# xwhan/ProQA

Hardware: AMD Instinct MI355X
Metric: queries/sec top-80 MIPS over 18M x 128 index (higher is better)
Workload: dtype int8 nomination + f16 re-scoring; 1 GPU; top-80 MIPS, 2032 q x 18000000 x 128 fp16 rows in HBM (BASELINE configs[2]; x1 row shards: co...; rows=18000000, queries=2032, topk=80, parallelism=corpus-row-shard x1, exchange=none, rounds=4, fallback_rounds=0, leap_rank=33, world_size=1

## Files before the change

### proqa_amd/csrc/mips_index.cpp

```cpp
#include <algorithm>
#include <cmath>
#include <cstdio>
#include <cstdlib>
#include <cstring>
#include <condition_variable>
#include <mutex>
#include <new>
#include <thread>
#include <vector>

#include <fcntl.h>
#include <unistd.h>
#include <cerrno>

#include "common.h"
#include "mips_kernels.h"

namespace proqa {

struct Slab {
  long long r0, r1;
};

}
// ... 119 lines not shown
  } pending;
};

namespace proqa {
namespace {

constexpr int kMaxRounds = kOverflowWords;

bool debug_flag(const char* name) { return getenv(name) != nullptr; }
const bool kDebugCand = debug_flag("PROQA_DEBUG_CAND");
const unsigned kFilterFlags = getenv("PROQA_FILTER_FLAGS") ? (unsigned)atoi(getenv("PROQA_FILTER_FLAGS")) : 0u;
const int kWideQw = getenv("PROQA_FILTER_QW") && (atoi(getenv("PROQA_FILTER_QW")) == 4 || atoi(getenv("PROQA_FILTER_QW")) == 1)
                        ? atoi(getenv("PROQA_FILTER_QW")) : 2;
const bool kDebugRounds = debug_flag("PROQA_DEBUG_ROUNDS");
const bool kDeepRing = getenv("PROQA_I8_DEEP_RING") && atoi(getenv("PROQA_I8_DEEP_RING")) != 0;
const bool kRowSplit = !(getenv("PROQA_I8_ROW_SPLIT") && atoi(getenv("PROQA_I8_ROW_SPLIT")) == 0);
const double kSmallMergeLimit = getenv("PROQA_NOM_SMALL_MERGE_LIMIT") ? atof(getenv("PROQA_NOM_SMALL_MERGE_LIMIT")) : 200.0;

int read_inexact(proqa_index* idx, const char* what, hipStream_t st, unsigned* n_inexact) {
  unsigned c[2] = {0, 0};
  PROQA_HIP(hipMemcpyAsync(c, idx->inexact, sizeof c, hipMemcpyDeviceToHost, st));
  PROQA_HIP(hipStreamSynchronize(st));
  if (c[1])
    return fail(PROQA_EINVAL, "%s: %u float32 values exceed the fp16 range (|x| > 65504); such embeddings are not "
                              "supported", what, c[1]);
  *n_inexact = c[0];
  return PROQA_OK;
}

int reserve_rows32(proqa_index* idx, int64_t rows) {
// ... 106 lines not shown
  if (idx->xb8) (void)hipFree(idx->xb8);
      idx->xb8 = nullptr;
      idx->q8_epoch = idx->rows_epoch;
      return PROQA_OK;
    }
    idx->capacity8 = cap;
  }
  PROQA_HIP(hipMemsetAsync(idx->qstats, 0, sizeof(QuantStats), st));
  PROQA_HIP(launch_column_stats(idx->xb, idx->n, idx->col_partial, idx->col, idx->qstats, st));
  PROQA_HIP(launch_quantise_rows_i8(idx->xb, idx->n, idx->col, idx->xb8, idx->blk8, idx->qstats, st));
  QuantStats h;
  PROQA_HIP(hipMemcpyAsync(&h, idx->qstats, sizeof h, hipMemcpyDeviceToHost, st));
  PROQA_HIP(hipStreamSynchronize(st));
  idx->q8_epoch = idx->rows_epoch;
  idx->q8_usable = h.nonfinite == 0u && h.max_inorm != 0u;
  return PROQA_OK;
}

constexpr int64_t kAddPieceRows = 1 << 20;
constexpr int kLoaderSlots = 4;
constexpr int64_t kLoaderPieceBytes = 8 << 20;

int ingest_f32_piece(proqa_index* idx, int64_t row, int64_t m, const void* src_host, bool pinned, hipStream_t st) {
  if (int rc = ensure_stage(idx, (size_t)kAddPieceRows * kDim * 4)) return rc;
  char* dst = idx->xb + (size_t)row * kDim * 2;
  if (pinned)
    PROQA_HIP(hipMemcpyAsync(idx->stage_dev, src_host, (size_t)m * kDim * 4, hipMemcpyHostToDevice, st));
  else
    PROQA_HIP(hipMemcpy(idx->stage_dev, src_host, (size_t)m * kDim * 4, hipMemcpyHostToDevice));
  PROQA_HIP(hipMemsetAsync(idx->inexact, 0, 2 * sizeof(unsigned), st));
// ... 1182 lines not shown
  PROQA_HIP(hipEventRecord(idx->ev[0], st));
  int fallback = 0;
  auto prep_first = [&]() -> int {
    const bool check_q = dtype == PROQA_F32;
    if (check_q) PROQA_HIP(hipMemsetAsync(idx->inexact, 0, 2 * sizeof(unsigned), st));
    PROQA_HIP(launch_prep_queries(xq_dev, dtype, nq, idx->ws_nq_pad, idx->xq_pad, idx->tau, idx->run_n, idx->stat_dev,
                                  nullptr, true, check_q ? idx->inexact : nullptr, idx->overflow, st, idx->short_rounds));
    if (check_q) {
      unsigned bad = 0;
      if (int rc = read_inexact(idx, "index_search (queries)", st, &bad)) return rc;
      if (bad && !idx->allow_rounding)
        if (int rc = enable_exact(idx, st)) return rc;
    }
    return PROQA_OK;
  };
  auto setup_nominate = [&]() -> int {
    if (!nomination_eligible(idx, k)) return PROQA_OK;
    if (idx->q8_epoch != idx->rows_epoch) {
      if (idx->q8_searches_on_copy > 1) idx->q8_short_lived_builds = 0;
      if (idx->nominate_mode == 1 && idx->q8_short_lived_builds >= 2 && idx->q8_seen_epoch != idx->rows_epoch) {
        idx->q8_seen_epoch = idx->rows_epoch;
        log_line("index %p: rows changed again after an int8 copy that served %d search(es): this search scans the fp16 rows, the "
                 "copy is rebuilt when the rows stay", (void*)idx, idx->q8_searches_on_copy);
        return PROQA_OK;
      }
      idx->q8_seen_epoch = idx->rows_epoch;
      if (defer) {
        idx->q8_build_due = true;
        return PROQA_OK;
      }
      if (int rc = ensure_q8(idx, st)) return rc;
    }
    if (!idx->q8_usable) return PROQA_OK;
    if (idx->q8_unprofitable && idx->nominate_mode != 2) {
      if (++idx->q8_suspended_searches < idx->q8_probe_after) return PROQA_OK;
      log_line("index %p: re-probing the int8 nomination scan after %d searches on the fp16 rows", (void*)idx,
               idx->q8_suspended_searches);
    }
    PROQA_HIP(launch_prep_queries_i8(idx->xq_pad, idx->ws_nq_pad, idx->col, idx->qstats, idx->xq8, idx->qparams, idx->stat_nom, st));
    idx->q8_active = true;
    ++idx->q8_searches_on_copy;
    return PROQA_OK;
  };
  if (one_pass.use) {
    if (int rc = prep_first()) return rc;
    bool done = false;
    if (!idx->exact)
      if (int rc = search_one_pass(idx, one_pass, qw, n_qtiles, nq, nq_pad, k, PageOut{D_dev, (long long*)I_dev, idx_offset, k, 0},
                                   st, &done))
        return rc;
    if (done) {
      idx->stats.candidates += (int64_t)idx->mirror->candidates;
      (void)hipEventElapsedTime(&idx->stats.total_ms, idx->ev[0], idx->ev[1]);
      return PROQA_OK;
    }
    if (!idx->exact) ++fallback;
  }
  const int n_pages = ceil_div<int>(k, page_size);
  if (defer && n_pages == 1 && !fallback) {
    if (int rc = prep_first()) return rc;
    if (idx->exact)
      PROQA_HIP(launch_query_margins(xq_dev, dtype, nq, idx->ws_nq_pad, idx->norm_stats, idx->xq32, idx->margin,
                                     idx->tau, idx->tau_filter, st));
    if (int rc = setup_nominate()) return rc;
    PagePlan plan;
    if (int rc = page_enqueue(idx, qw, n_qtiles, nq, nq_pad, k, false, PageOut{D_dev, (long long*)I_dev, idx_offset, k, 0}, st, true,
                              &plan, status_dev))
      return rc;
    proqa_index::Pending& pe = idx->pending;
    pe.active = true;
    pe.qw = qw;
    pe.n_qtiles = n_qtiles;
    pe.nq = nq;
    pe.nq_pad = nq_pad;
    pe.k = k;
    pe.dtype = dtype;
    pe.xq_dev = xq_dev;
    pe.D = D_dev;
    pe.I = (long long*)I_dev;
    pe.idx_offset = idx_offset;
    pe.st = st;
    pe.slabs.swap(plan.slabs);
    pe.boot = plan.boot;
    return PROQA_OK;
  }
  if (n_pages > 1) PROQA_HIP(hipMemsetAsync(idx->done, 0, (size_t)idx->ws_nq_pad, st));
  for (int p = 0; p < n_pages; ++p) {
    const int page_k = std::min(page_size, k - p * page_size);
    if (p == 0) {
      if (int rc = prep_first()) return rc;
      if (n_pages == 1 && !fallback)
        if (int rc = setup_nominate()) return rc;
    } else {
      PROQA_HIP(launch_prep_queries(xq_dev, dtype, nq, idx->ws_nq_pad, idx->xq_pad, idx->tau, idx->run_n, idx->stat_dev,
                                    idx->done, false, nullptr, idx->overflow, st));
    }
    if (idx->exact)
      PROQA_HIP(launch_query_margins(xq_dev, dtype, nq, idx->ws_nq_pad, idx->norm_stats, idx->xq32, idx->margin,
                                     idx->tau, idx->tau_filter, st));
    const PageOut out{D_dev, (long long*)I_dev, idx_offset, k, p * page_size};
    bool boot_overflow = false;
    if (int rc = search_page(idx, qw, n_qtiles, nq, nq_pad, page_k, p > 0, out, st, &fallback, true, &boot_overflow)) return rc;
    if (boot_overflow) {
      PROQA_HIP(launch_prep_queries(xq_dev, dtype, nq, idx->ws_nq_pad, idx->xq_pad, idx->tau, idx->run_n, idx->stat_dev,
                                    nullptr, true, nullptr, idx->overflow, st));
      ++fallback;
      if (int rc = search_page(idx, qw, n_qtiles, nq, nq_pad, page_k, false, out, st, &fallback, false, &boot_overflow))
// ... 480 lines not shown
  if ((long long)n_parts * k >= (1ll << 27))
    return fail(PROQA_EINVAL, "topk_merge_device: n_parts*k=%lld is too large", (long long)n_parts * k);
  if (stride_d < nq * k || stride_i < nq * k)
    return fail(PROQA_EINVAL, "topk_merge_device: part strides %lld / %lld are shorter than a part (%lld)", (long long)stride_d,
                (long long)stride_i, (long long)(nq * k));
  PROQA_HIP(launch_merge_lists(D_parts_dev, (const long long*)I_parts_dev, n_parts, nq, k, (long long)stride_d, (long long)stride_i,
                               D_dev, (long long*)I_dev, as_stream(stream), nullptr, 0, nullptr, false));
  return PROQA_OK;
}

int proqa_topk_merge_device(const float* D_parts_dev, const int64_t* I_parts_dev, int n_parts, int64_t nq,
                            int k, float* D_dev, int64_t* I_dev, void* stream) {
  return proqa_topk_merge_strided_device(D_parts_dev, I_parts_dev, n_parts, nq, k, nq * k, nq * k, D_dev, I_dev, stream);
}

}
```

### proqa_amd/csrc/mips_kernels.h

```cpp
#pragma once
#include <hip/hip_runtime.h>
#include <stdint.h>

#include "../../include/proqa_hip.h"

namespace proqa {

constexpr int kDim = PROQA_EMBED_DIM;
constexpr int kFilterWaves = 8;
constexpr int kFilterThreads = kFilterWaves * 64;
__host__ __device__ constexpr unsigned filter_tile_queries(int qw) { return (qw == 4 ? 4u : 8u) * (unsigned)qw * 32u; }
constexpr int kStageRows = 128;
constexpr int kMergeThreads = 256;
constexpr int kMaxMergeListKeys = 16384;
constexpr int kMaxSortKeys = 2048;
constexpr int kPageK = kMaxSortKeys / 2;
constexpr int kBigSortKeys = 8192;
constexpr int kMidSortKeys = 4096;
constexpr int kBigPageK = kBigSortKeys / 2;
constexpr int kOnePassSortKeys = 16384;
constexpr int kOnePassMergeThreads = 1024;
constexpr int kOnePassLaneCap = 24;
constexpr int kLaneCap = 8;
constexpr int kBigLaneCap = 32;
// ... 65 lines not shown
  int compact;
  int nom_keys;
  const void* xq16;
  const char* xb16;
  unsigned long long* stat_nominated;
  int next_rank;
  int leap_check;
  unsigned* short_rounds;
  int round_bit;
};

constexpr int kStageBytesI8 = kStageRows * kDim;
struct NominateParams {
  float off;
  float inv_unit;
  float margin_r;
  float err_norm;
};
static_assert(sizeof(NominateParams) == 16, "one 16-byte load per lane");
struct QuantStats {
  unsigned max_resid;
  unsigned max_inorm;
  unsigned max_xnorm;
  unsigned nonfinite;
};
struct FilterArgsI8 {
  const signed char* xq8;
  const signed char* xb8;
  long long slab_row0;
  long long slab_row1;
  int rows_per_chunk;
  const float* tau;
  const NominateParams* qp;
  const float2* blk;
  CandidateStore store;
  unsigned* overflow;
  unsigned flags;
  unsigned q_blocks;
};
hipError_t launch_filter_i8(const FilterArgsI8& a, int qw, unsigned grid, hipStream_t st, bool deep = false);
constexpr int kColStatGroups = 1024;
hipError_t launch_column_stats(const void* xb16, long long n, float* partial, float* col, QuantStats* stats, hipStream_t st);
hipError_t launch_quantise_rows_i8(const void* xb16, long long n, const float* col, signed char* xb8, float2* blk, QuantStats* stats,
                                   hipStream_t st);
hipError_t launch_prep_queries_i8(const void* xq_pad16, long long nq_pad, const float* col, const QuantStats* stats,
                                  signed char* xq8, NominateParams* qp, unsigned long long* stat_nom, hipStream_t st);

hipError_t launch_filter(const FilterArgs& a, int qw, bool inclusive, unsigned grid, hipStream_t st);
#ifdef PROQA_FILTER_STAMPS
void read_filter_stamps(unsigned long long* out5);
#endif
hipError_t launch_advance_page(const unsigned long long* run_keys, const unsigned* run_n, long long nq, int page_k,
                               unsigned long long* bound_keys, float* ub, unsigned char* done, const float* margin,
                               float* ub_filter, hipStream_t st);
hipError_t launch_merge(const MergeArgs& a, unsigned nq_pad, hipStream_t st);
hipError_t launch_gather_index_rows(const void* xb16, const float* xb32, long long n_index, const long long* ids, long long n,
                                    long long idx_offset, void* out, bool out_f32, hipStream_t st);
hipError_t launch_flag_short_lists(const unsigned* run_n, long long nq, unsigned want, unsigned* flag, hipStream_t st);
hipError_t launch_bootstrap(const char* xb, const void* xq_pad, int n_rows, unsigned nq_pad, int k, float* scores,
                            unsigned long long* run_keys, unsigned* run_n, float* tau, unsigned long long* stat,
                            unsigned* overflow, hipStream_t st, int run_stride = 0, int tau_rank = 0);
// ... 42 lines not shown
```

### proqa_amd/csrc/mips_kernels.hip

```cpp
#include <hip/hip_runtime.h>
#include <algorithm>
#include <hipcub/hipcub.hpp>
#include <stdint.h>
#include <stdlib.h>

#include <type_traits>

#include "common.h"
#include "mips_kernels.h"

namespace proqa {
namespace {

typedef _Float16 f16x8 __attribute__((ext_vector_type(8)));
typedef float f32x16 __attribute__((ext_vector_type(16)));
typedef float f32x4 __attribute__((ext_vector_type(4)));

constexpr int kRowBytes = kDim * 2;
constexpr int kStageBytes = kStageRows * kRowBytes;
constexpr int kSubRows = 32;
#ifndef PROQA_DMA_AUX
#define PROQA_DMA_AUX 2
#endif
constexpr int kDmaAux = PROQA_DMA_AUX;
// ... 411 lines not shown
}

typedef int i32x4 __attribute__((ext_vector_type(4)));
typedef int i32x16 __attribute__((ext_vector_type(16)));
constexpr int kRowBytesI8 = kDim;
constexpr int kSubBytesI8 = kSubRows * kRowBytesI8;

__device__ __forceinline__ int imax(int a, int b) { return a > b ? a : b; }
__device__ __forceinline__ int max16_i32(const i32x16& v) {
  const int m0 = imax(imax(v[0], v[1]), v[2]), m1 = imax(imax(v[3], v[4]), v[5]), m2 = imax(imax(v[6], v[7]), v[8]),
            m3 = imax(imax(v[9], v[10]), v[11]), m4 = imax(imax(v[12], v[13]), v[14]);
  return imax(imax(imax(m0, m1), m2), imax(imax(m3, m4), v[15]));
}

struct LaneThreshold {
  float A, B, E;
};
__device__ __forceinline__ LaneThreshold lane_threshold(float tau, const NominateParams& p) {
  LaneThreshold t;
  t.B = p.margin_r;
  t.E = p.err_norm;
  if (!(tau > -__builtin_inff())) {
    t.A = -__builtin_inff();
  } else if (tau == __builtin_inff()) {
    t.A = __builtin_inff();
  } else {
    const float a = (tau - p.off) * p.inv_unit;
    t.A = a - __builtin_fabsf(a) * 0x1p-20f;
  }
  return t;
}
__device__ __forceinline__ float block_threshold(const LaneThreshold& t, float G, float X) {
  return __builtin_fmaf(-t.E, X, __builtin_fmaf(t.A, G, -t.B));
}

__device__ __forceinline__ unsigned nominee_mask(const i32x16& acc, float thr) {
  const int ti = thr < -2147483000.f ? (int)0x80000000 : (int)__builtin_floorf(thr);
  unsigned mask = 0u;
#define PROQA_BIT(n) "v_cmp_gt_i32 vcc, %" #n ", %17\n\tv_addc_co_u32 %0, vcc, %0, %0, vcc\n\t"
  asm volatile(PROQA_BIT(16) PROQA_BIT(15) PROQA_BIT(14) PROQA_BIT(13) PROQA_BIT(12) PROQA_BIT(11) PROQA_BIT(10) PROQA_BIT(9)
               PROQA_BIT(8) PROQA_BIT(7) PROQA_BIT(6) PROQA_BIT(5) PROQA_BIT(4) PROQA_BIT(3) PROQA_BIT(2) PROQA_BIT(1)
               : "+v"(mask)
               : "v"(acc[0]), "v"(acc[1]), "v"(acc[2]), "v"(acc[3]), "v"(acc[4]), "v"(acc[5]), "v"(acc[6]), "v"(acc[7]), "v"(acc[8]),
                 "v"(acc[9]), "v"(acc[10]), "v"(acc[11]), "v"(acc[12]), "v"(acc[13]), "v"(acc[14]), "v"(acc[15]), "v"(ti)
               : "vcc");
#undef PROQA_BIT
  return mask;
}
// ... 315 lines not shown
    const float* p = partial + (size_t)g * 3 * kDim;
    sum += (double)p[d];
    lo = __builtin_fminf(lo, p[kDim + d]);
    hi = __builtin_fmaxf(hi, p[2 * kDim + d]);
  }
  const float mean = (float)(sum / (double)(n > 0 ? n : 1));
  const float c = __builtin_fmaxf(hi - mean, mean - lo);
  const bool finite = c >= 0.f && c < __builtin_inff() && mean == mean;
  const float inv = finite && c > 0.f ? 1.0f / c : 0.f;
  if (!finite || !(inv < __builtin_inff())) atomicOr(&stats->nonfinite, 1u);
  col[d] = finite ? mean : 0.f;
  col[kDim + d] = inv;
  col[2 * kDim + d] = finite ? c : 0.f;
}

__global__ __launch_bounds__(256) void quantise_rows_i8(const _Float16* __restrict__ xb, long long n, const float* __restrict__ col,
                                                        signed char* __restrict__ xb8, float2* __restrict__ blk,
                                                        QuantStats* __restrict__ stats) {
  const int lane = threadIdx.x & 63;
  const int sub = lane & 15, rsub = lane >> 4;
  float mu[8], inv[8];
#pragma unroll
  for (int e = 0; e < 8; ++e) {
    mu[e] = col[sub * 8 + e];
    inv[e] = col[kDim + sub * 8 + e];
  }
  float max_r = 0.f, max_i = 0.f, max_x = 0.f;
  const long long n_blocks = (n + 31) / 32;
  for (long long b = (long long)blockIdx.x * 4 + (threadIdx.x >> 6); b < n_blocks; b += (long long)gridDim.x * 4) {
    float u[8][8];
    float amax = 0.f, sx_max = 0.f;
#pragma unroll
    for (int it = 0; it < 8; ++it) {
      const long long row = b * 32 + it * 4 + rsub;
      f16x8 v = {0};
      const bool live = row < n;
      if (live) v = *(const f16x8*)(xb + row * kDim + sub * 8);
      float sx = 0.f;
#pragma unroll
      for (int e = 0; e < 8; ++e) {
        const float x = (float)v[e];
        u[it][e] = live ? (x - mu[e]) * inv[e] : 0.f;
// ... 20 lines not shown
        const float i = __builtin_fminf(127.f, __builtin_fmaxf(-127.f, __builtin_rintf(t)));
        const float r = t - i;
        o[e] = (signed char)(int)i;
        sr += r * r;
        si += i * i;
      }
      if (row < n) *(i8x8*)(xb8 + row * kDim + sub * 8) = o;
#pragma unroll
      for (int off = 8; off > 0; off >>= 1) {
        sr += __shfl_xor(sr, off, 64);
        si += __shfl_xor(si, off, 64);
      }
      sr_max = sr > sr_max ? sr : sr_max;
      si_max = si > si_max ? si : si_max;
    }
    const float xb_ = __builtin_sqrtf(wave_max_f(si_max)) * (1.0f + 0x1p-10f);
    if (lane == 0) blk[b] = make_float2(G, xb_);
    max_r = sr_max > max_r ? sr_max : max_r;
    max_i = si_max > max_i ? si_max : max_i;
    max_x = sx_max > max_x ? sx_max : max_x;
  }
  max_r = wave_max_f(max_r);
  max_i = wave_max_f(max_i);
  max_x = wave_max_f(max_x);
  if (lane == 0) {
    const float r = __builtin_sqrtf(max_r) * (1.0f + 0x1p-10f), i = __builtin_sqrtf(max_i) * (1.0f + 0x1p-10f),
                x = __builtin_sqrtf(max_x) * (1.0f + 0x1p-10f);
    if (r > 0.f) atomicMax(&stats->max_resid, __float_as_uint(r));
    if (i > 0.f) atomicMax(&stats->max_inorm, __float_as_uint(i));
    if (x > 0.f) atomicMax(&stats->max_xnorm, __float_as_uint(x));
  }
}

__global__ __launch_bounds__(256) void prep_queries_i8(const _Float16* __restrict__ xq, long long nq_pad, const float* __restrict__ col,
                                                       const QuantStats* __restrict__ stats, signed char* __restrict__ xq8,
                                                       NominateParams* __restrict__ qp, unsigned long long* __restrict__ stat_nom) {
  const int lane = threadIdx.x & 63;
  const long long q = (long long)blockIdx.x * 4 + (threadIdx.x >> 6);
  if (q >= nq_pad) return;
  const float q0 = (float)xq[q * kDim + 2 * lane], q1 = (float)xq[q * kDim + 2 * lane + 1];
  const float mu0 = col[2 * lane], mu1 = col[2 * lane + 1];
  const float w0 = q0 * col[2 * kDim + 2 * lane], w1 = q1 * col[2 * kDim + 2 * lane + 1];
  const float wmax = wave_max_f(__builtin_fmaxf(__builtin_fabsf(w0), __builtin_fabsf(w1)));
  const float s_q = wmax / 127.0f;
  const bool ok = s_q > 0.f && s_q < __builtin_inff();
  const float inv = ok ? 1.0f / s_q : 0.f;
  const float u0 = w0 * inv, u1 = w1 * inv;
  const float i0 = __builtin_fminf(127.f, __builtin_fmaxf(-127.f, __builtin_rintf(u0)));
  const float i1 = __builtin_fminf(127.f, __builtin_fmaxf(-127.f, __builtin_rintf(u1)));
  typedef signed char i8x2 __attribute__((ext_vector_type(2)));
  const i8x2 o = {(signed char)(int)i0, (signed char)(int)i1};
  *(i8x2*)(xq8 + q * kDim + 2 * lane) = o;
  const float e0 = u0 - i0, e1 = u1 - i1;
  const float n_u = __builtin_sqrtf(wave_sum_f(u0 * u0 + u1 * u1)) * (1.0f + 0x1p-10f);
  const float n_e = __builtin_sqrtf(wave_sum_f(e0 * e0 + e1 * e1)) * (1.0f + 0x1p-10f) + 0x1p-10f;
  const float n_q = __builtin_sqrtf(wave_sum_f(q0 * q0 + q1 * q1)) * (1.0f + 0x1p-10f);
  const float abs_off = wave_sum_f(__builtin_fabsf(q0 * mu0) + __builtin_fabsf(q1 * mu1));
  double off = (double)q0 * (double)mu0 + (double)q1 * (double)mu1;
#pragma unroll
  for (int d = 32; d > 0; d >>= 1) off += __shfl_xor(off, d, 64);
  if (lane == 0) {
    const float R = __uint_as_float(stats->max_resid) + 0x1p-10f, Xf = __uint_as_float(stats->max_xnorm);
    const float delta = 0x1p-14f * n_q * Xf + 0x1p-20f * abs_off;
    NominateParams p;
    p.off = (float)off + delta + __builtin_fabsf((float)off) * 0x1p-22f;
    p.inv_unit = inv;
    p.margin_r = n_u * R * (1.0f + 0x1p-10f) + 0x1p-6f;
    p.err_norm = n_e;
    if (!(stats->nonfinite == 0u)) p.margin_r = __builtin_inff();
    qp[q] = p;
    stat_nom[q] = 0ull;
  }
}

__device__ __forceinline__ float filter_threshold(float t, float margin) {
  if (!(t > -__builtin_inff())) return t;
  return t - margin - __builtin_fabsf(t) * 0x1p-21f;
}

struct ExactCtx {
  unsigned* nom;
  unsigned* n_nom;
};

__device__ __forceinline__ void keep_scores_regs(const uint4 (&src)[5], unsigned q, bool inclusive,
                                                 unsigned long long bound, const ExactCtx& ex,
                                                 unsigned long long* keys, unsigned* n_keys, unsigned cap) {
// ... 765 lines not shown
  unsigned n = s_n_keys;
  if (n > kCompactKeys) {
    if (tid == 0) *a.overflow = 1u;
    n = kCompactKeys;
  }
  unsigned long long* dst = (unsigned long long*)(a.out.lane_log + lane_list_index(a.out, g >> 1, q, (int)(g & 1)) * a.out.lane_cap);
  if ((unsigned)tid < n) dst[tid] = s_keys[tid];
  if (tid == 0) {
    a.out.lane_cnt[lane_cnt_index(a.out, g >> 1, q, (int)(g & 1))] = n;
    if (a.stat_nominated) atomicAdd(a.stat_nominated + q, (unsigned long long)n_nom);
  }
}

constexpr int kBootWaves = 4;
constexpr int kBootTilesPerWave = 4;
__global__ __launch_bounds__(kBootWaves * 64) void bootstrap_scores(const char* __restrict__ xb, const void* __restrict__ xq,
                                                                    int n_rows, int s_stride, float* __restrict__ S) {
  __shared__ float tile[kBootWaves][32][33];
  const int lane = threadIdx.x & 63;
  const int wave = __builtin_amdgcn_readfirstlane(threadIdx.x >> 6);
  const int li = lane & 31, half = lane >> 5;
  const unsigned q0 = blockIdx.y * 32;
  const char* bp = (const char*)xq + (size_t)(q0 + li) * kRowBytes;
  f16x8 qf[8];
#pragma unroll
  for (int j = 0; j < 8; ++j) qf[j] = *(const f16x8*)(bp + (2 * j + half) * 16);
  f16x8 af[kBootTilesPerWave][8];
#pragma unroll
  for (int t = 0; t < kBootTilesPerWave; ++t) {
    const int row0 = ((blockIdx.x * kBootTilesPerWave + t) * kBootWaves + wave) * 32;
    const int arow = row0 + li < n_rows ? row0 + li : n_rows - 1;
    const char* ap = xb + (size_t)arow * kRowBytes;
#pragma unroll
    for (int j = 0; j < 8; ++j) af[t][j] = *(const f16x8*)(ap + (2 * j + half) * 16);
  }
#pragma unroll
  for (int t = 0; t < kBootTilesPerWave; ++t) {
    const int row0 = ((blockIdx.x * kBootTilesPerWave + t) * kBootWaves + wave) * 32;
    if (row0 >= n_rows) break;
    f32x16 acc = {0};
#pragma unroll
    for (int j = 0; j < 8; ++j) acc = __builtin_amdgcn_mfma_f32_32x32x16_f16(af[t][j], qf[j], acc, 0, 0, 0);
#pragma unroll
    for (int r = 0; r < 16; ++r) tile[wave][li][(r & 3) + 8 * (r >> 2) + 4 * half] = acc[r];
#pragma unroll
    for (int i = 0; i < 16; ++i) {
      const int qq = 2 * i + half;
      if (row0 + li < n_rows) S[(size_t)(q0 + qq) * s_stride + row0 + li] = tile[wave][qq][li];
    }
  }
}

template <int E>
__global__ __launch_bounds__(kMergeThreads) void bootstrap_select(const float* __restrict__ S, int n_rows, int s_stride,
                                                                  int k, int run_stride, unsigned long long* __restrict__ run_keys,
                                                                  unsigned* __restrict__ run_n, float* __restrict__ tau,
                                                                  unsigned long long* __restrict__ stat_candidates,
                                                                  unsigned* __restrict__ overflow, int tau_rank) {
  __shared__ __attribute__((aligned(16))) unsigned long long keys[kMaxSortKeys];
  __shared__ unsigned long long s_bound;
  __shared__ unsigned s_n_keys;
  const unsigned q = blockIdx.x;
  const int tid = threadIdx.x;
// ... 92 lines not shown
    float v = 0.f;
    if (q < nq) v = dtype == PROQA_F16 ? (float)((const _Float16*)xq)[i] : ((const float*)xq)[i];
    const _Float16 hq = (_Float16)v;
    xq_pad[i] = hq;
    if (inexact && (float)hq != v && v == v) {
      atomicAdd(inexact, 1u);
      if (__builtin_isinf((float)hq) && !__builtin_isinf(v)) atomicAdd(inexact + 1, 1u);
    }
  }
  if (i < nq_pad) {
    const bool live = i < nq && !debug_nohit && !(done && done[i]);
    tau[i] = live ? -__builtin_inff() : (debug_nohit && i < nq ? 3.0e38f : __builtin_inff());
    run_n[i] = 0;
    if (reset_stat) stat[i] = 0;
  }
}

__global__ __launch_bounds__(256) void finalize_topk(const unsigned long long* run_keys, const unsigned* run_n, long long nq,
                                                     int k, long long idx_offset, float* D, long long* I, int out_stride,
                                                     int out_offset, const unsigned* overflow, unsigned* status,
                                                     SearchMirror* mirror, const unsigned long long* stat,
                                                     const unsigned long long* stat_nominated) {
  if (blockIdx.x == 0 && (status || mirror)) {
    __shared__ unsigned long long s_part[8];
    bool any = false;
    for (int w = threadIdx.x; w < kOverflowWords; w += 256) {
      const unsigned v = overflow[w];
      if (mirror) mirror->overflow[w] = v;
      any = any || v != 0u;
    }
// ... 388 lines not shown
    return hipErrorInvalidValue;
  return hipGetLastError();
}

hipError_t launch_column_stats(const void* xb16, long long n, float* partial, float* col, QuantStats* stats, hipStream_t st) {
  hipLaunchKernelGGL(column_stats_partial, dim3(kColStatGroups), dim3(256), 0, st, (const _Float16*)xb16, n, partial, stats);
  hipLaunchKernelGGL(column_stats_finish, dim3(1), dim3(kDim), 0, st, partial, kColStatGroups, n, col, stats);
  return hipGetLastError();
}

hipError_t launch_quantise_rows_i8(const void* xb16, long long n, const float* col, signed char* xb8, float2* blk, QuantStats* stats,
                                   hipStream_t st) {
  if (n == 0) return hipSuccess;
  const long long want = ((n + 31) / 32 + 3) / 4;
  const unsigned grid = (unsigned)std::min<long long>(want, 8ll * 1024);
  hipLaunchKernelGGL(quantise_rows_i8, dim3(grid), dim3(256), 0, st, (const _Float16*)xb16, n, col, xb8, blk, stats);
  return hipGetLastError();
}

hipError_t launch_prep_queries_i8(const void* xq_pad16, long long nq_pad, const float* col, const QuantStats* stats,
                                  signed char* xq8, NominateParams* qp, unsigned long long* stat_nom, hipStream_t st) {
  if (nq_pad == 0) return hipSuccess;
  hipLaunchKernelGGL(prep_queries_i8, dim3((unsigned)((nq_pad + 3) / 4)), dim3(256), 0, st, (const _Float16*)xq_pad16, nq_pad, col,
                     stats, xq8, qp, stat_nom);
  return hipGetLastError();
}

#ifdef PROQA_FILTER_STAMPS
void read_filter_stamps(unsigned long long* out5) {
  (void)hipDeviceSynchronize();
// ... 31 lines not shown
                                float* xq32, float* margin, const float* tau, float* tau_filter, hipStream_t st) {
  if (nq_pad == 0) return hipSuccess;
  hipLaunchKernelGGL(query_margins, dim3((unsigned)((nq_pad + 3) / 4)), dim3(256), 0, st, xq, dtype, nq, nq_pad,
                     norm_stats, xq32, margin, tau, tau_filter);
  return hipGetLastError();
}

hipError_t launch_bootstrap(const char* xb, const void* xq_pad, int n_rows, unsigned nq_pad, int k, float* scores,
                            unsigned long long* run_keys, unsigned* run_n, float* tau, unsigned long long* stat,
                            unsigned* overflow, hipStream_t st, int run_stride, int tau_rank) {
  if (run_stride <= 0) run_stride = k;
  if (tau_rank <= 0 || tau_rank > k) tau_rank = k;
  const int s_stride = (n_rows + 31) / 32 * 32;
  const unsigned row_tiles = (unsigned)(s_stride / 32);
  const unsigned per_wg = kBootWaves * kBootTilesPerWave;
  hipLaunchKernelGGL(bootstrap_scores, dim3((row_tiles + per_wg - 1) / per_wg, nq_pad / 32), dim3(kBootWaves * 64), 0, st,
                     xb, xq_pad, n_rows, s_stride, scores);
#define PROQA_SELECT_CASE(E)                                                                                            \
  hipLaunchKernelGGL(bootstrap_select<E>, dim3(nq_pad), dim3(kMergeThreads), 0, st, scores, n_rows, s_stride, k, run_stride, \
                     run_keys, run_n, tau, stat, overflow, tau_rank)
  if (n_rows <= 4 * kMergeThreads)
    PROQA_SELECT_CASE(4);
  else if (n_rows <= 8 * kMergeThreads)
    PROQA_SELECT_CASE(8);
  else if (n_rows <= 16 * kMergeThreads)
    PROQA_SELECT_CASE(16);
  else
    PROQA_SELECT_CASE(32);
#undef PROQA_SELECT_CASE
  static_assert(kBootstrapMaxRows == 32 * kMergeThreads, "largest select");
  return hipGetLastError();
// ... 61 lines not shown
    else
      hipLaunchKernelGGL((topk_merge<kMergeF16, kMaxSortKeys>), dim3(nq_pad), dim3(kMergeThreads), 0, st, a);
  }
  return hipGetLastError();
}

static const bool kDebugNoHit = getenv("PROQA_DEBUG_NOHIT") != nullptr;

hipError_t launch_prep_queries(const void* xq, int dtype, long long nq, long long nq_pad, void* xq_pad,
                               float* tau, unsigned* run_n, unsigned long long* stat, const unsigned char* done,
                               bool reset_stat, unsigned* inexact, unsigned* overflow, hipStream_t st, unsigned* short_rounds) {
  const long long n = nq_pad * kDim;
  hipLaunchKernelGGL(prep_queries, dim3((unsigned)((n + 255) / 256)), dim3(256), 0, st, xq, dtype, nq, nq_pad,
                     (_Float16*)xq_pad, tau, run_n, stat, done, reset_stat ? 1 : 0, inexact,
                     kDebugNoHit ? 1 : 0, overflow, short_rounds);
  return hipGetLastError();
}

hipError_t launch_finalize(const unsigned long long* run_keys, const unsigned* run_n, long long nq, int page_k,
                           long long idx_offset, float* D, long long* I, int out_stride, int out_offset,
                           const unsigned* overflow, unsigned* status, SearchMirror* mirror, const unsigned long long* stat,
                           hipStream_t st, const unsigned long long* stat_nominated) {
  const long long n = nq * page_k;
  if (n == 0) return hipSuccess;
  hipLaunchKernelGGL(finalize_topk, dim3((unsigned)((n + 255) / 256)), dim3(256), 0, st, run_keys, run_n,
                     nq, page_k, idx_offset, D, I, out_stride, out_offset, overflow, status, mirror, stat, stat_nominated);
  return hipGetLastError();
}

hipError_t launch_merge_lists(const float* D_parts, const long long* I_parts, int n_parts, long long nq,
// ... 91 lines not shown
```

Baseline: 485,400 queries/s.

## Tighten int8 nomination bound with kappa, fuse query prep, widen bootstrap query tiles

Replaces the int8 nomination error bound with a per-block term that combines the row norm and a kappa-scaled residual. Kappa is the median norm ratio measured on sampled rows by a new kernel, and the tighter bound is meant to let fewer false nominees through to fp16 re-scoring. It also fuses fp16 query padding with int8 query quantisation into one kernel to save a launch and a pass over the queries. Separately, bootstrap_scores now handles two 32-query blocks per workgroup to reuse the loaded row fragments. It adds debug entry points for reading device state, and the correctness of the new bound depends on the kappa estimate being a valid bound.

```diff
diff --git a/proqa_amd/csrc/mips_index.cpp b/proqa_amd/csrc/mips_index.cpp
--- a/proqa_amd/csrc/mips_index.cpp
+++ b/proqa_amd/csrc/mips_index.cpp
@@ -157,6 +157,7 @@
                         ? atoi(getenv("PROQA_FILTER_QW")) : 2;
 const bool kDebugRounds = debug_flag("PROQA_DEBUG_ROUNDS");
 const bool kDeepRing = getenv("PROQA_I8_DEEP_RING") && atoi(getenv("PROQA_I8_DEEP_RING")) != 0;
+const bool kFusedPrep = !(getenv("PROQA_FUSED_PREP") && atoi(getenv("PROQA_FUSED_PREP")) == 0);
 const bool kRowSplit = !(getenv("PROQA_I8_ROW_SPLIT") && atoi(getenv("PROQA_I8_ROW_SPLIT")) == 0);
 const double kSmallMergeLimit = getenv("PROQA_NOM_SMALL_MERGE_LIMIT") ? atof(getenv("PROQA_NOM_SMALL_MERGE_LIMIT")) : 200.0;
 
@@ -293,6 +294,13 @@
   PROQA_HIP(hipStreamSynchronize(st));
   idx->q8_epoch = idx->rows_epoch;
   idx->q8_usable = h.nonfinite == 0u && h.max_inorm != 0u;
+  {
+    float f[4];
+    const unsigned w[4] = {h.kappa, h.max_resid, ~h.min_inorm_c, h.max_inorm};
+    std::memcpy(f, w, sizeof f);
+    log_line("index %p: int8 copy of %lld rows: kappa %.1f (median ||w/s|| / ||e|| of its own rows as queries), largest row residual "
+             "%.3f, block norms X_b in [%.1f, %.1f]", (void*)idx, (long long)idx->n, f[0], f[1], f[2], f[3]);
+  }
   return PROQA_OK;
 }
 
@@ -1505,7 +1513,8 @@
     }
     return PROQA_OK;
   };
-  auto setup_nominate = [&]() -> int {
+  auto decide_nominate = [&](bool* want) -> int {
+    *want = false;
     if (!nomination_eligible(idx, k)) return PROQA_OK;
     if (idx->q8_epoch != idx->rows_epoch) {
       if (idx->q8_searches_on_copy > 1) idx->q8_short_lived_builds = 0;
@@ -1528,9 +1537,36 @@
       log_line("index %p: re-probing the int8 nomination scan after %d searches on the fp16 rows", (void*)idx,
                idx->q8_suspended_searches);
     }
-    PROQA_HIP(launch_prep_queries_i8(idx->xq_pad, idx->ws_nq_pad, idx->col, idx->qstats, idx->xq8, idx->qparams, idx->stat_nom, st));
-    idx->q8_active = true;
-    ++idx->q8_searches_on_copy;
+    *want = true;
+    return PROQA_OK;
+  };
+  auto prep_page0 = [&](bool nominate) -> int {
+    bool want = false;
+    const bool fusable = nominate && kFusedPrep && (dtype == PROQA_F16 || idx->allow_rounding);
+    if (fusable)
+      if (int rc = decide_nominate(&want)) return rc;
+    if (fusable && want) {
+      const bool check_q = dtype == PROQA_F32;
+      if (check_q) PROQA_HIP(hipMemsetAsync(idx->inexact, 0, 2 * sizeof(unsigned), st));
+      PROQA_HIP(launch_prep_queries_fused(xq_dev, dtype, nq, idx->ws_nq_pad, idx->xq_pad, idx->tau, idx->run_n, idx->stat_dev,
+                                          check_q ? idx->inexact : nullptr, idx->overflow, idx->short_rounds, idx->col, idx->qstats,
+                                          idx->xq8, idx->qparams, idx->stat_nom, st));
+      if (check_q) {
+        unsigned bad = 0;
+        if (int rc = read_inexact(idx, "index_search (queries)", st, &bad)) return rc;
+      }
+    } else {
+      if (int rc = prep_first()) return rc;
+      if (nominate && !fusable)
+        if (int rc = decide_nominate(&want)) return rc;
+      if (want)
+        PROQA_HIP(launch_prep_queries_i8(idx->xq_pad, idx->ws_nq_pad, idx->col, idx->qstats, idx->xq8, idx->qparams, idx->stat_nom,
+                                         st));
+    }
+    if (want) {
+      idx->q8_active = true;
+      ++idx->q8_searches_on_copy;
+    }
     return PROQA_OK;
   };
   if (one_pass.use) {
@@ -1549,11 +1585,10 @@
   }
   const int n_pages = ceil_div<int>(k, page_size);
   if (defer && n_pages == 1 && !fallback) {
-    if (int rc = prep_first()) return rc;
+    if (int rc = prep_page0(true)) return rc;
     if (idx->exact)
       PROQA_HIP(launch_query_margins(xq_dev, dtype, nq, idx->ws_nq_pad, idx->norm_stats, idx->xq32, idx->margin,
                                      idx->tau, idx->tau_filter, st));
-    if (int rc = setup_nominate()) return rc;
     PagePlan plan;
     if (int rc = page_enqueue(idx, qw, n_qtiles, nq, nq_pad, k, false, PageOut{D_dev, (long long*)I_dev, idx_offset, k, 0}, st, true,
                               &plan, status_dev))
@@ -1579,9 +1614,7 @@
   for (int p = 0; p < n_pages; ++p) {
     const int page_k = std::min(page_size, k - p * page_size);
     if (p == 0) {
-      if (int rc = prep_first()) return rc;
-      if (n_pages == 1 && !fallback)
-        if (int rc = setup_nominate()) return rc;
+      if (int rc = prep_page0(n_pages == 1 && !fallback)) return rc;
     } else {
       PROQA_HIP(launch_prep_queries(xq_dev, dtype, nq, idx->ws_nq_pad, idx->xq_pad, idx->tau, idx->run_n, idx->stat_dev,
                                     idx->done, false, nullptr, idx->overflow, st));
@@ -2092,4 +2125,40 @@
   return proqa_topk_merge_strided_device(D_parts_dev, I_parts_dev, n_parts, nq, k, nq * k, nq * k, D_dev, I_dev, stream);
 }
 
-}
+int proqa_dev_prep_queries(proqa_index* idx, const void* xq_dev, int64_t nq, int dtype, int fused, void* stream) {
+  if (!idx || !xq_dev || nq <= 0) return fail(PROQA_EINVAL, "dev_prep_queries: bad argument");
+  if (dtype != PROQA_F16 && dtype != PROQA_F32) return fail(PROQA_EINVAL, "dev_prep_queries: bad dtype %d", dtype);
+  hipStream_t st = as_stream(stream);
+  if (int rc = ensure_workspace(idx, round_up<int64_t>(nq, 512), 1)) return rc;
+  if (int rc = ensure_q8(idx, st)) return rc;
+  if (!idx->xb8 || !idx->q8_usable) return fail(PROQA_EINVAL, "dev_prep_queries: the index has no usable int8 copy");
+  if (fused) {
+    PROQA_HIP(launch_prep_queries_fused(xq_dev, dtype, nq, idx->ws_nq_pad, idx->xq_pad, idx->tau, idx->run_n, idx->stat_dev, nullptr,
+                                        idx->overflow, idx->short_rounds, idx->col, idx->qstats, idx->xq8, idx->qparams,
+                                        idx->stat_nom, st));
+  } else {
+    PROQA_HIP(launch_prep_queries(xq_dev, dtype, nq, idx->ws_nq_pad, idx->xq_pad, idx->tau, idx->run_n, idx->stat_dev, nullptr, true,
+                                  nullptr, idx->overflow, st, idx->short_rounds));
+    PROQA_HIP(launch_prep_queries_i8(idx->xq_pad, idx->ws_nq_pad, idx->col, idx->qstats, idx->xq8, idx->qparams, idx->stat_nom, st));
+  }
+  PROQA_HIP(hipStreamSynchronize(st));
+  return PROQA_OK;
+}
+
+int proqa_dev_read_state(proqa_index* idx, int which, void* dst, int64_t* bytes) {
+  if (!idx || !dst || !bytes) return fail(PROQA_EINVAL, "dev_read_state: NULL argument");
+  const size_t q = (size_t)idx->ws_nq_pad;
+  const void* src[9] = {idx->xq_pad, idx->xq8, idx->qparams, idx->tau, idx->run_n, idx->stat_dev, idx->stat_nom, idx->short_rounds,
+                        idx->overflow};
+  const size_t size[9] = {q * kDim * 2, q * kDim, q * sizeof(NominateParams), q * sizeof(float), q * sizeof(unsigned),
+                          q * sizeof(unsigned long long), q * sizeof(unsigned long long), q * sizeof(unsigned),
+                          kOverflowWords * sizeof(unsigned)};
+  if (which < 0 || which >= 9 || !src[which]) return fail(PROQA_EINVAL, "dev_read_state: nothing to read for %d", which);
+  if ((size_t)*bytes < size[which]) return fail(PROQA_EINVAL, "dev_read_state: %zu bytes needed", size[which]);
+  PROQA_HIP(hipDeviceSynchronize());
+  PROQA_HIP(hipMemcpy(dst, src[which], size[which], hipMemcpyDeviceToHost));
+  *bytes = (int64_t)size[which];
+  return PROQA_OK;
+}
+
+}
diff --git a/proqa_amd/csrc/mips_kernels.h b/proqa_amd/csrc/mips_kernels.h
--- a/proqa_amd/csrc/mips_kernels.h
+++ b/proqa_amd/csrc/mips_kernels.h
@@ -103,8 +103,8 @@
 struct NominateParams {
   float off;
   float inv_unit;
-  float margin_r;
-  float err_norm;
+  float bias;
+  float coef;
 };
 static_assert(sizeof(NominateParams) == 16, "one 16-byte load per lane");
 struct QuantStats {
@@ -112,6 +112,8 @@
   unsigned max_inorm;
   unsigned max_xnorm;
   unsigned nonfinite;
+  unsigned min_inorm_c;
+  unsigned kappa;
 };
 struct FilterArgsI8 {
   const signed char* xq8;
@@ -134,6 +136,11 @@
                                    hipStream_t st);
 hipError_t launch_prep_queries_i8(const void* xq_pad16, long long nq_pad, const float* col, const QuantStats* stats,
                                   signed char* xq8, NominateParams* qp, unsigned long long* stat_nom, hipStream_t st);
+
+hipError_t launch_prep_queries_fused(const void* xq, int dtype, long long nq, long long nq_pad, void* xq_pad, float* tau,
+                                     unsigned* run_n, unsigned long long* stat, unsigned* inexact, unsigned* overflow,
+                                     unsigned* short_rounds, const float* col, const QuantStats* stats, signed char* xq8,
+                                     NominateParams* qp, unsigned long long* stat_nom, hipStream_t st);
 
 hipError_t launch_filter(const FilterArgs& a, int qw, bool inclusive, unsigned grid, hipStream_t st);
 #ifdef PROQA_FILTER_STAMPS
diff --git a/proqa_amd/csrc/mips_kernels.hip b/proqa_amd/csrc/mips_kernels.hip
--- a/proqa_amd/csrc/mips_kernels.hip
+++ b/proqa_amd/csrc/mips_kernels.hip
@@ -449,12 +449,12 @@
 }
 
 struct LaneThreshold {
-  float A, B, E;
+  float A, D, C;
 };
 __device__ __forceinline__ LaneThreshold lane_threshold(float tau, const NominateParams& p) {
   LaneThreshold t;
-  t.B = p.margin_r;
-  t.E = p.err_norm;
+  t.D = p.bias;
+  t.C = p.coef;
   if (!(tau > -__builtin_inff())) {
     t.A = -__builtin_inff();
   } else if (tau == __builtin_inff()) {
@@ -465,8 +465,8 @@
   }
   return t;
 }
-__device__ __forceinline__ float block_threshold(const LaneThreshold& t, float G, float X) {
-  return __builtin_fmaf(-t.E, X, __builtin_fmaf(t.A, G, -t.B));
+__device__ __forceinline__ float block_threshold(const LaneThreshold& t, float G, float Z) {
+  return __builtin_fmaf(-t.C, Z, __builtin_fmaf(t.A, G, -t.D));
 }
 
 __device__ __forceinline__ unsigned nominee_mask(const i32x16& acc, float thr) {
@@ -812,6 +812,42 @@
   col[2 * kDim + d] = finite ? c : 0.f;
 }
 
+__global__ __launch_bounds__(256) void nominate_kappa(const _Float16* __restrict__ xb, long long n, const float* __restrict__ col,
+                                                      QuantStats* __restrict__ stats) {
+  __shared__ float s_ratio[256];
+  const int lane = threadIdx.x & 63, wave = threadIdx.x >> 6;
+  const int m = (int)(n < 256 ? n : 256);
+  const float c0 = col[2 * kDim + 2 * lane], c1 = col[2 * kDim + 2 * lane + 1];
+  for (int i = wave; i < 256; i += 4) {
+    float ratio = -1.f;
+    if (i < m) {
+      const long long row = (long long)i * (n / m);
+      const float w0 = (float)xb[row * kDim + 2 * lane] * c0, w1 = (float)xb[row * kDim + 2 * lane + 1] * c1;
+      const float s = wave_max_f(__builtin_fmaxf(__builtin_fabsf(w0), __builtin_fabsf(w1))) / 127.0f;
+      const float inv = s > 0.f && s < __builtin_inff() ? 1.0f / s : 0.f;
+      const float u0 = w0 * inv, u1 = w1 * inv;
+      const float e0 = u0 - __builtin_rintf(u0), e1 = u1 - __builtin_rintf(u1);
+      const float n_u = __builtin_sqrtf(wave_sum_f(u0 * u0 + u1 * u1)), n_e = __builtin_sqrtf(wave_sum_f(e0 * e0 + e1 * e1));
+      if (n_u > 0.f && n_e > 0x1p-10f && n_u / n_e < __builtin_inff()) ratio = n_u / n_e;
+    }
+    if (lane == 0) s_ratio[i] = ratio;
+  }
+  __syncthreads();
+  const int t = threadIdx.x;
+  const float mine = s_ratio[t];
+  int below = 0, valid = 0;
+  for (int j = 0; j < 256; ++j) {
+    const float r = s_ratio[j];
+    valid += r > 0.f;
+    below += r > 0.f && (r < mine || (r == mine && j < t));
+  }
+  if (valid == 0) {
+    if (t == 0) stats->kappa = __float_as_uint(160.0f);
+  } else if (mine > 0.f && below == valid / 2) {
+    stats->kappa = __float_as_uint(__builtin_fminf(65536.f, __builtin_fmaxf(1.0f, mine)));
+  }
+}
+
 __global__ __launch_bounds__(256) void quantise_rows_i8(const _Float16* __restrict__ xb, long long n, const float* __restrict__ col,
                                                         signed char* __restrict__ xb8, float2* __restrict__ blk,
                                                         QuantStats* __restrict__ stats) {
@@ -823,7 +859,8 @@
     mu[e] = col[sub * 8 + e];
     inv[e] = col[kDim + sub * 8 + e];
   }
-  float max_r = 0.f, max_i = 0.f, max_x = 0.f;
+  float max_r = 0.f, max_i = 0.f, max_x = 0.f, min_i = __builtin_inff();
+  const float kappa = __uint_as_float(stats->kappa) * (1.0f + 0x1p-10f);
   const long long n_blocks = (n + 31) / 32;
   for (long long b = (long long)blockIdx.x * 4 + (threadIdx.x >> 6); b < n_blocks; b += (long long)gridDim.x * 4) {
     float u[8][8];
@@ -874,10 +911,13 @@
       sr_max = sr > sr_max ? sr : sr_max;
       si_max = si > si_max ? si : si_max;
     }
-    const float xb_ = __builtin_sqrtf(wave_max_f(si_max)) * (1.0f + 0x1p-10f);
-    if (lane == 0) blk[b] = make_float2(G, xb_);
+    si_max = wave_max_f(si_max);
+    const float xb_ = __builtin_sqrtf(si_max) * (1.0f + 0x1p-10f);
+    const float rb_ = __builtin_sqrtf(wave_max_f(sr_max)) * (1.0f + 0x1p-10f) + 0x1p-10f;
+    if (lane == 0) blk[b] = make_float2(G, __builtin_fmaf(kappa, rb_, xb_) * (1.0f + 0x1p-20f));
     max_r = sr_max > max_r ? sr_max : max_r;
     max_i = si_max > max_i ? si_max : max_i;
+    min_i = si_max < min_i ? si_max : min_i;
     max_x = sx_max > max_x ? sx_max : max_x;
   }
   max_r = wave_max_f(max_r);
@@ -889,16 +929,13 @@
     if (r > 0.f) atomicMax(&stats->max_resid, __float_as_uint(r));
     if (i > 0.f) atomicMax(&stats->max_inorm, __float_as_uint(i));
     if (x > 0.f) atomicMax(&stats->max_xnorm, __float_as_uint(x));
-  }
-}
-
-__global__ __launch_bounds__(256) void prep_queries_i8(const _Float16* __restrict__ xq, long long nq_pad, const float* __restrict__ col,
-                                                       const QuantStats* __restrict__ stats, signed char* __restrict__ xq8,
-                                                       NominateParams* __restrict__ qp, unsigned long long* __restrict__ stat_nom) {
-  const int lane = threadIdx.x & 63;
-  const long long q = (long long)blockIdx.x * 4 + (threadIdx.x >> 6);
-  if (q >= nq_pad) return;
-  const float q0 = (float)xq[q * kDim + 2 * lane], q1 = (float)xq[q * kDim + 2 * lane + 1];
+    if (min_i < __builtin_inff()) atomicMax(&stats->min_inorm_c, ~__float_as_uint(__builtin_sqrtf(min_i) * (1.0f - 0x1p-10f)));
+  }
+}
+
+__device__ __forceinline__ void quantise_query(int lane, long long q, float q0, float q1, const float* __restrict__ col,
+                                               const QuantStats* __restrict__ stats, signed char* __restrict__ xq8,
+                                               NominateParams* __restrict__ qp, unsigned long long* __restrict__ stat_nom) {
   const float mu0 = col[2 * lane], mu1 = col[2 * lane + 1];
   const float w0 = q0 * col[2 * kDim + 2 * lane], w1 = q1 * col[2 * kDim + 2 * lane + 1];
   const float wmax = wave_max_f(__builtin_fmaxf(__builtin_fabsf(w0), __builtin_fabsf(w1)));
@@ -920,17 +957,30 @@
 #pragma unroll
   for (int d = 32; d > 0; d >>= 1) off += __shfl_xor(off, d, 64);
   if (lane == 0) {
-    const float R = __uint_as_float(stats->max_resid) + 0x1p-10f, Xf = __uint_as_float(stats->max_xnorm);
+    const float Xf = __uint_as_float(stats->max_xnorm);
     const float delta = 0x1p-14f * n_q * Xf + 0x1p-20f * abs_off;
     NominateParams p;
     p.off = (float)off + delta + __builtin_fabsf((float)off) * 0x1p-22f;
     p.inv_unit = inv;
-    p.margin_r = n_u * R * (1.0f + 0x1p-10f) + 0x1p-6f;
-    p.err_norm = n_e;
-    if (!(stats->nonfinite == 0u)) p.margin_r = __builtin_inff();
+    const float x_max = __uint_as_float(stats->max_inorm);
+    float x_min = __uint_as_float(~stats->min_inorm_c);
+    if (!(x_min >= 0.f && x_min <= x_max)) x_min = 0.f;
+    const float C = n_u / __uint_as_float(stats->kappa) * (1.0f + 0x1p-10f);
+    const float d = (n_e - C) * (n_e > C ? x_max : x_min);
+    p.coef = C;
+    p.bias = d + __builtin_fabsf(d) * 0x1p-10f + 0x1p-6f;
+    if (!(stats->nonfinite == 0u)) p.bias = __builtin_inff();
     qp[q] = p;
     stat_nom[q] = 0ull;
   }
+}
+__global__ __launch_bounds__(256) void prep_queries_i8(const _Float16* __restrict__ xq, long long nq_pad, const float* __restrict__ col,
+                                                       const QuantStats* __restrict__ stats, signed char* __restrict__ xq8,
+                                                       NominateParams* __restrict__ qp, unsigned long long* __restrict__ stat_nom) {
+  const int lane = threadIdx.x & 63;
+  const long long q = (long long)blockIdx.x * 4 + (threadIdx.x >> 6);
+  if (q >= nq_pad) return;
+  quantise_query(lane, q, (float)xq[q * kDim + 2 * lane], (float)xq[q * kDim + 2 * lane + 1], col, stats, xq8, qp, stat_nom);
 }
 
 __device__ __forceinline__ float filter_threshold(float t, float margin) {
@@ -1726,17 +1776,21 @@
 
 constexpr int kBootWaves = 4;
 constexpr int kBootTilesPerWave = 4;
+constexpr int kBootQueryBlocks = 2;
 __global__ __launch_bounds__(kBootWaves * 64) void bootstrap_scores(const char* __restrict__ xb, const void* __restrict__ xq,
                                                                     int n_rows, int s_stride, float* __restrict__ S) {
   __shared__ float tile[kBootWaves][32][33];
   const int lane = threadIdx.x & 63;
   const int wave = __builtin_amdgcn_readfirstlane(threadIdx.x >> 6);
   const int li = lane & 31, half = lane >> 5;
-  const unsigned q0 = blockIdx.y * 32;
-  const char* bp = (const char*)xq + (size_t)(q0 + li) * kRowBytes;
-  f16x8 qf[8];
-#pragma unroll
-  for (int j = 0; j < 8; ++j) qf[j] = *(const f16x8*)(bp + (2 * j + half) * 16);
+  const unsigned q0 = blockIdx.y * (kBootQueryBlocks * 32);
+  f16x8 qf[kBootQueryBlocks][8];
+#pragma unroll
+  for (int qb = 0; qb < kBootQueryBlocks; ++qb) {
+    const char* bp = (const char*)xq + (size_t)(q0 + qb * 32 + li) * kRowBytes;
+#pragma unroll
+    for (int j = 0; j < 8; ++j) qf[qb][j] = *(const f16x8*)(bp + (2 * j + half) * 16);
+  }
   f16x8 af[kBootTilesPerWave][8];
 #pragma unroll
   for (int t = 0; t < kBootTilesPerWave; ++t) {
@@ -1750,15 +1804,24 @@
   for (int t = 0; t < kBootTilesPerWave; ++t) {
     const int row0 = ((blockIdx.x * kBootTilesPerWave + t) * kBootWaves + wave) * 32;
     if (row0 >= n_rows) break;
-    f32x16 acc = {0};
-#pragma unroll
-    for (int j = 0; j < 8; ++j) acc = __builtin_amdgcn_mfma_f32_32x32x16_f16(af[t][j], qf[j], acc, 0, 0, 0);
-#pragma unroll
-    for (int r = 0; r < 16; ++r) tile[wave][li][(r & 3) + 8 * (r >> 2) + 4 * half] = acc[r];
-#pragma unroll
-    for (int i = 0; i < 16; ++i) {
-      const int qq = 2 * i + half;
-      if (row0 + li < n_rows) S[(size_t)(q0 + qq) * s_stride + row0 + li] = tile[wave][qq][li];
+    f32x16 acc[kBootQueryBlocks];
+#pragma unroll
+    for (int qb = 0; qb < kBootQueryBlocks; ++qb) acc[qb] = f32x16{0};
+#pragma unroll
+    for (int j = 0; j < 8; ++j) {
+#pragma unroll
+      for (int qb = 0; qb < kBootQueryBlocks; ++qb)
+        acc[qb] = __builtin_amdgcn_mfma_f32_32x32x16_f16(af[t][j], qf[qb][j], acc[qb], 0, 0, 0);
+    }
+#pragma unroll
+    for (int qb = 0; qb < kBootQueryBlocks; ++qb) {
+#pragma unroll
+      for (int r = 0; r < 16; ++r) tile[wave][li][(r & 3) + 8 * (r >> 2) + 4 * half] = acc[qb][r];
+#pragma unroll
+      for (int i = 0; i < 16; ++i) {
+        const int qq = 2 * i + half;
+        if (row0 + li < n_rows) S[(size_t)(q0 + qb * 32 + qq) * s_stride + row0 + li] = tile[wave][qq][li];
+      }
     }
   }
 }
@@ -1881,6 +1944,47 @@
     run_n[i] = 0;
     if (reset_stat) stat[i] = 0;
   }
+}
+
+__global__ __launch_bounds__(256) void prep_queries_fused(const void* __restrict__ xq, int dtype, long long nq, long long nq_pad,
+                                                          _Float16* __restrict__ xq_pad, float* __restrict__ tau,
+                                                          unsigned* __restrict__ run_n, unsigned long long* __restrict__ stat,
+                                                          unsigned* inexact, int debug_nohit, unsigned* __restrict__ overflow,
+                                                          unsigned* __restrict__ short_rounds, const float* __restrict__ col,
+                                                          const QuantStats* __restrict__ stats, signed char* __restrict__ xq8,
+                                                          NominateParams* __restrict__ qp, unsigned long long* __restrict__ stat_nom) {
+  if (blockIdx.x == 0 && threadIdx.x < kOverflowWords) overflow[threadIdx.x] = 0u;
+  const int lane = threadIdx.x & 63;
+  const long long q = (long long)blockIdx.x * 4 + (threadIdx.x >> 6);
+  if (q >= nq_pad) return;
+  float v[2] = {0.f, 0.f};
+  if (q < nq) {
+#pragma unroll
+    for (int e = 0; e < 2; ++e) {
+      const long long i = q * kDim + 2 * lane + e;
+      v[e] = dtype == PROQA_F16 ? (float)((const _Float16*)xq)[i] : ((const float*)xq)[i];
+    }
+  }
+  typedef _Float16 f16x2_t __attribute__((ext_vector_type(2)));
+  const f16x2_t h = {(_Float16)v[0], (_Float16)v[1]};
+  *(f16x2_t*)(xq_pad + q * kDim + 2 * lane) = h;
+  if (inexact) {
+#pragma unroll
+    for (int e = 0; e < 2; ++e) {
+      if ((float)h[e] != v[e] && v[e] == v[e]) {
+        atomicAdd(inexact, 1u);
+        if (__builtin_isinf((float)h[e]) && !__builtin_isinf(v[e])) atomicAdd(inexact + 1, 1u);
+      }
+    }
+  }
+  if (lane == 0) {
+    const bool live = q < nq && !debug_nohit;
+    tau[q] = live ? -__builtin_inff() : (debug_nohit && q < nq ? 3.0e38f : __builtin_inff());
+    run_n[q] = 0;
+    stat[q] = 0;
+    short_rounds[q] = 0u;
+  }
+  quantise_query(lane, q, (float)h[0], (float)h[1], col, stats, xq8, qp, stat_nom);
 }
 
 __global__ __launch_bounds__(256) void finalize_topk(const unsigned long long* run_keys, const unsigned* run_n, long long nq,
@@ -2299,6 +2403,7 @@
   if (n == 0) return hipSuccess;
   const long long want = ((n + 31) / 32 + 3) / 4;
   const unsigned grid = (unsigned)std::min<long long>(want, 8ll * 1024);
+  hipLaunchKernelGGL(nominate_kappa, dim3(1), dim3(256), 0, st, (const _Float16*)xb16, n, col, stats);
   hipLaunchKernelGGL(quantise_rows_i8, dim3(grid), dim3(256), 0, st, (const _Float16*)xb16, n, col, xb8, blk, stats);
   return hipGetLastError();
 }
@@ -2360,7 +2465,7 @@
   const int s_stride = (n_rows + 31) / 32 * 32;
   const unsigned row_tiles = (unsigned)(s_stride / 32);
   const unsigned per_wg = kBootWaves * kBootTilesPerWave;
-  hipLaunchKernelGGL(bootstrap_scores, dim3((row_tiles + per_wg - 1) / per_wg, nq_pad / 32), dim3(kBootWaves * 64), 0, st,
+  hipLaunchKernelGGL(bootstrap_scores, dim3((row_tiles + per_wg - 1) / per_wg, nq_pad / (32 * kBootQueryBlocks)), dim3(kBootWaves * 64), 0, st,
                      xb, xq_pad, n_rows, s_stride, scores);
 #define PROQA_SELECT_CASE(E)                                                                                            \
   hipLaunchKernelGGL(bootstrap_select<E>, dim3(nq_pad), dim3(kMergeThreads), 0, st, scores, n_rows, s_stride, k, run_stride, \
@@ -2452,6 +2557,17 @@
   hipLaunchKernelGGL(prep_queries, dim3((unsigned)((n + 255) / 256)), dim3(256), 0, st, xq, dtype, nq, nq_pad,
                      (_Float16*)xq_pad, tau, run_n, stat, done, reset_stat ? 1 : 0, inexact,
                      kDebugNoHit ? 1 : 0, overflow, short_rounds);
+  return hipGetLastError();
+}
+
+hipError_t launch_prep_queries_fused(const void* xq, int dtype, long long nq, long long nq_pad, void* xq_pad, float* tau,
+                                     unsigned* run_n, unsigned long long* stat, unsigned* inexact, unsigned* overflow,
+                                     unsigned* short_rounds, const float* col, const QuantStats* stats, signed char* xq8,
+                                     NominateParams* qp, unsigned long long* stat_nom, hipStream_t st) {
+  if (nq_pad == 0) return hipSuccess;
+  hipLaunchKernelGGL(prep_queries_fused, dim3((unsigned)((nq_pad + 3) / 4)), dim3(256), 0, st, xq, dtype, nq, nq_pad,
+                     (_Float16*)xq_pad, tau, run_n, stat, inexact, kDebugNoHit ? 1 : 0, overflow, short_rounds, col, stats, xq8, qp,
+                     stat_nom);
   return hipGetLastError();
 }
 
```

New measurement: 487,100 queries/s (median of 6 runs). Within noise of the previous version (+0.4%).
